# ghar1821/Chronoclust

Measured on AMD Instinct MI355X. Metric: points clustered/sec (20-dim), higher is better.
Workload: dtype f64; 1 GPU; C2: 1 timepoint, 1000000x20 synthetic blobs (seed 42+rank), 5000 microclusters; exact sequential semantics; online + offline phases per step; one independent st; points=1000000, dim=20, microclusters=5000, clusters=5000, streams=1

## Files before the change

chronoclust_amd/csrc/cc_api.hip:

```cpp
#include <hip/hip_runtime.h>

#include <algorithm>
#include <chrono>
#include <cmath>
#include <cstdio>
#include <cstdlib>
#include <cstring>
#include <limits>
#include <optional>
#include <string>
#include <thread>
#include <type_traits>
#include <vector>

#include "../../include/chronoclust_hip.h"
#include "cc_comm.h"
#include "cc_common.h"
#include "cc_csv.h"
#include "cc_offline.h"
#include "cc_online.h"
#include "cc_assign.h"
#include "cc_policy.h"
#include "cc_batch.h"

#include "cc_handle.h"

namespace {


template <int DP, bool DIRTY>
void launch_scan_dp(cc_handle* h, hipStream_t st, int win, Rows rows, const Cand* clean, Cand* part, int S, int round,
                    int mode, int shard_rank, int shard_world, int phase);

template <int DP>
int scan_u_wgs_per_cu()
{
    constexpr int NW = ScanShape<DP, false>::NW;
    static int blocks = 0;
    static const bool ok = hipOccupancyMaxActiveBlocksPerMultiprocessor(&blocks, k_scan_u<DP, NW>, 64 * NW, 0) == hipSuccess && blocks >= 1;
    return ok ? blocks : ScanUShape<DP>::WGS;
}

template <int DP>
ScanPlan scan_plan_dp(const cc_handle* h)
{
    ScanPlan p;
    p.dp = DP;
    const cc::ScanWidth w = cc::scan_width(h->d, h->hc.filter != 0, h->hc.pow2 != 0);
    p.scan_u = h->allow_scan_u && w.scan_u;
    p.pad_rows = p.scan_u && h->d != DP;
    if (p.scan_u && w.chain == CC_CHAIN_COMMON) p.chain = ScanPlan::COMMON;
    else if (h->allow_scan_p3 && h->allow_prune_general && !h->tainted && w.chain == CC_CHAIN_GENERAL) p.chain = ScanPlan::GENERAL;
    const bool p3 = h->allow_scan_p3 && DP <= 40;
    p.form = p3 ? ScanPlan::P3 : (h->allow_scan_p2 && DP <= 40 ? ScanPlan::P2 : ScanPlan::P1);
    if (p.chain == ScanPlan::COMMON && h->split_a_mode == 2) p.split_rows = 0;
    else if (p.chain == ScanPlan::COMMON && h->split_a_mode == 1 && !p3) p.split_rows = 10000;
    p.listed_rows = h->p3_listed_rows;
    const bool p3_sized = p3 && h->split_a_mode != 2;
    p.seed16 = h->allow_seed16 && (p.chain == ScanPlan::GENERAL || p3_sized);
    p.prune_applicable = p.chain != ScanPlan::NONE ? 1 : 0;
    p.allow_guess = (h->allow_guess && p.chain != ScanPlan::GENERAL) ? (h->allow_lean ? 1 : 2) : 0;
    p.allow_probe = (h->allow_probe && p.chain != ScanPlan::GENERAL) ? 1 : 0;
    p.force_prune_rows = (p.prune_applicable && h->allow_seed16 && p3_sized) ? h->force_prune_rows : 0;
    p.waves = ScanShape<DP, false>::NW;
    p.dirty_waves = ScanShape<DP, true>::NW;
    p.plain_wgs_per_cu = p.scan_u ? scan_u_wgs_per_cu<DP>() : ScanShape<DP, false>::WGS;
    p.prune_wgs_per_cu = h->prune_rounds4 > 0 ? h->prune_rounds4 : (DP <= 20 ? (p3_sized ? 8 : 16) : 24);
    return p;
}

ScanPlan scan_plan(const cc_handle* h)
{
    switch (cc::scan_width(h->d, false, false).padded) {
    case 4: return scan_plan_dp<4>(h);
    case 8: return scan_plan_dp<8>(h);
    case 14: return scan_plan_dp<14>(h);
    case 16: return scan_plan_dp<16>(h);
    case 20: return scan_plan_dp<20>(h);
    case 32: return scan_plan_dp<32>(h);
    case 40: return scan_plan_dp<40>(h);
    default: return scan_plan_dp<64>(h);
    }
}

template <int DP>
struct ScanCall {
    static constexpr int NW = ScanShape<DP, false>::NW;
    cc_handle* h; hipStream_t st; const Rows& rows;
    int round, mode, win, S;
    Cand* part;

    void scan_u(int n_pts, int srank, int sworld, const int* plist) const
    {
        hipLaunchKernelGGL((k_scan_u<DP, NW>), dim3((n_pts + 63) / 64, S), dim3(64 * NW), 0, st, h->ctl.p, h->Xt.p, rows.cen,
                           rows.scl, rows.kind, rows.key, part, round, mode, h->part_stride, srank, sworld, plist);
    }
    void prefix16() const
    {
        ensure_prefix16(h);
        const size_t a16_rows = h->tab.cap + 2 * CC_P16_TM;
        hipLaunchKernelGGL((k_prefix16<DP>), dim3((unsigned)((a16_rows + 255) / 256)), dim3(256), 0, st, (const Ctl*)h->ctl.p,
                           rows.cen, rows.kind, h->a16.p, h->hdr16.p, h->a16_stride, round, mode);
    }
    void seeds(int n_pts, int Sp, const int* plist, bool s16) const
    {
        const dim3 grid((n_pts + 127) / 128, Sp), block(64 * NW);
        if (s16) {
            if constexpr (DP <= 40) {
                hipLaunchKernelGGL((k_seed16<DP, NW>), grid, block, 0, st, (const Ctl*)h->ctl.p, (const double*)h->Xt.p, rows.cen, h->spart.p,
                                   round, mode, h->spart_stride, (const cc_h8*)h->a16.p, (const Prefix16Hdr*)h->hdr16.p, h->a16_stride);
                ++h->stats.seed16_launches;
            } else {
                throw HipErr{hipErrorInvalidValue, "k_seed16 is compiled up to 40 dimensions"};
            }
        } else {
            hipLaunchKernelGGL((k_seed<DP, NW>), grid, block, 0, st, h->ctl.p, h->Xt.p, rows.cen, rows.kind, h->spart.p, round, mode,
                               h->spart_stride, h->cmax.p, plist);
        }
        hipLaunchKernelGGL((k_seed_merge<DP>), dim3((2 * n_pts + 63) / 64), dim3(64), 0, st, h->ctl.p, h->X.p, rows.cen, rows.scl, h->spart.p,
                           h->spart_stride, Sp, h->thr.p, h->thr32.p, h->thr_stride, s16 ? 0.0 : h->prune_F, round, mode, h->cmax.p,
                           h->pstat_p(), plist, h->d);
    }
    template <bool LISTED, bool GENERAL>
    void scan_p3(unsigned lds, int srank, int sworld, double gF, unsigned long long* found) const
    {
        hipLaunchKernelGGL((k_scan_p3<DP, NW, LISTED, GENERAL>), dim3((win + 127) / 128, S), dim3(64 * NW), lds, st, h->ctl.p, h->Xt.p,
                           rows.cen, rows.scl, rows.kind, rows.key, h->thr.p, h->thr_stride, part, round, mode, h->part_stride, srank,
                           sworld, h->pstat_p(), gF, found, (const cc_h8*)h->a16.p, (const Prefix16Hdr*)h->hdr16.p, h->a16_stride,
                           GENERAL ? (const double*)h->X.p : nullptr, GENERAL ? rows.cf1 : nullptr, GENERAL ? rows.cf2 : nullptr,
                           GENERAL ? rows.w : nullptr);
    }
    void scan_p(int n_pts, int Sp, Cand* p, size_t p_stride, int srank, int sworld, const int* plist, double gF,
                unsigned long long* found) const
    {
        hipLaunchKernelGGL((k_scan_p<DP, NW, false>), dim3((n_pts + 63) / 64, Sp), dim3(64 * NW), 0, st, h->ctl.p, h->Xt.p, rows.cen,
                           rows.scl, rows.kind, rows.key, h->thr.p, h->thr32.p, h->thr_stride, p, round, mode, p_stride, srank, sworld,
                           h->pstat_p(), plist, gF, found, (const unsigned*)nullptr, (size_t)0, 0, 1);
    }
    void scan_split(int srank, int sworld, double gF, unsigned long long* found) const
    {
        const int nsub = S * NW;
        const int tps = cc_mask_tiles_per_sub((int)std::min<size_t>(h->tab.cap, (size_t)INT_MAX - 64), nsub);
        const size_t need = (size_t)((win + 127) / 128) * (size_t)nsub * (size_t)tps;
        if (need > h->mask_stride) { h->masks.ensure(2 * need); h->mask_stride = need; }
        hipLaunchKernelGGL((k_scan_a<DP, NW>), dim3((win + 127) / 128, S), dim3(64 * NW), 0, st, (const Ctl*)h->ctl.p,
                           (const double*)h->Xt.p, rows.cen, rows.kind, (const double*)h->thr.p, h->thr_stride, h->masks.p,
                           h->mask_stride, tps, round, mode, srank, sworld, gF);
        int q = 1;
        const int tiles = (win + 63) / 64;
        const int resident = h->n_cus * (DP <= 20 ? CC_SCANP_WGS20 : (DP <= 40 ? 3 : 2));
        for (int c = 1; c <= S; ++c)
            if (S % c == 0 && 2 * tiles * (S / c) >= 3 * resident) q = c;
        static const int q_env = []() { const char* e = getenv("CHRONOCLUST_HIP_SCANB_Q"); return e ? atoi(e) : 0; }();
        if (q_env > 0 && S % q_env == 0) q = q_env;
        hipLaunchKernelGGL((k_scan_p<DP, NW, true>), dim3(tiles, S / q), dim3(64 * NW), 0, st, h->ctl.p, h->Xt.p, rows.cen, rows.scl,
                           rows.kind, rows.key, h->thr.p, h->thr32.p, h->thr_stride, part, round, mode, h->part_stride, srank, sworld,
                           h->pstat_p(), (const int*)nullptr, gF, found, (const unsigned*)h->masks.p, h->mask_stride, tps, q);
    }
};

template <int DP, bool DIRTY>
void launch_scan_dp(cc_handle* h, hipStream_t st, int win, Rows rows, const Cand* clean, Cand* part, int S, int round,
                    int mode, int shard_rank, int shard_world, int phase)
{
    constexpr int NW = ScanShape<DP, DIRTY>::NW;
    const dim3 block(64 * NW);
    constexpr int TILE = 64 * ScanShape<DP, DIRTY>::PT;
    const dim3 grid((win + TILE - 1) / TILE, S);
    if constexpr (!DIRTY) {
        static_assert(ScanShape<DP, false>::PT == 1, "k_scan_u holds one window point per lane");
        const ScanPlan& pl = h->scan_plan;
        const ScanCall<DP> L{h, st, rows, round, mode, win, S, part};
        if (pl.scan_u) ++h->stats.scan_u_launches;
        if constexpr (DP > 8) {
            auto window_scan = [&](int srank, int sworld, double gF, unsigned long long* found, bool have_prefix16) {
                if (pl.split(h->hc.m_rows)) return L.scan_split(srank, sworld, gF, found);
                if constexpr (DP <= 40) {
                    if (pl.form == ScanPlan::P3) {
                        if (!have_prefix16) L.prefix16();
                        const bool listed = pl.listed(h->hc.m_rows);
                        if (pl.chain == ScanPlan::GENERAL) {
                            if (listed) L.template scan_p3<true, true>(0, srank, sworld, gF, found);
                            else L.template scan_p3<false, true>(0, srank, sworld, gF, found);
                        } else {
                            static const char* const lds_kb = getenv("CHRONOCLUST_HIP_SCAN_LDS_KB");
                            static const unsigned p3_lds = lds_kb ? (unsigned)atoi(lds_kb) * 1024u : 0u;
                            if (listed) L.template scan_p3<true, false>(p3_lds, srank, sworld, gF, found);
                            else L.template scan_p3<false, false>(p3_lds, srank, sworld, gF, found);
                        }
                        ++h->stats.scan_p2_launches;
                        return;
                    }
                    if (pl.form == ScanPlan::P2) {
                        hipLaunchKernelGGL((k_scan_p2<DP, NW>), dim3((win + 127) / 128, S), block, 0, st, h->ctl.p, h->Xt.p, rows.cen, rows.scl,
                                           rows.kind, rows.key, h->thr.p, h->thr_stride, part, round, mode, h->part_stride, srank, sworld,
                                           h->pstat_p(), gF, found);
                        ++h->stats.scan_p2_launches;
                        return;
                    }
                }
                L.scan_p(win, S, part, h->part_stride, srank, sworld, nullptr, gF, found);
            };
            auto seeded_chain = [&](int n_pts, const int* plist, Cand* p, size_t p_stride, int Sp, int srank, int sworld) {
                const bool whole_window = plist == nullptr && n_pts == win && p_stride == h->part_stride && Sp == S;
                const bool s16 = whole_window && pl.seed16;
                const bool have_prefix16 = whole_window && (s16 || pl.chain == ScanPlan::GENERAL);
                if constexpr (DP <= 40) if (have_prefix16) L.prefix16();
                L.seeds(n_pts, Sp, plist, s16);
                if (whole_window) window_scan(srank, sworld, 0.0, nullptr, have_prefix16);
                else L.scan_p(n_pts, Sp, p, p_stride, srank, sworld, plist, 0.0, nullptr);
            };
            auto missed_scan = [&](const int* list) {
                if (!h->allow_missed_plain) return seeded_chain(CC_MISSED_CAP, list, part, h->part_stride, S, shard_rank, shard_world);
                ++h->stats.missed_plain_launches;
                L.scan_u(CC_MISSED_CAP, shard_rank, shard_world, list);
            };
            if (pl.chain == ScanPlan::GENERAL && h->prune_now && phase == 0) {
                ++h->stats.scan_p_launches;
                return seeded_chain(win, nullptr, part, h->part_stride, S, shard_rank, shard_world);
            }
            if (pl.chain == ScanPlan::COMMON) {
                if (phase == 1) {
                    hipLaunchKernelGGL(k_missed_g, dim3(1), dim3(1024), 0, st, h->ctl.p, (const Cand*)h->gpart.p, h->gpart_stride,
                                       (size_t)win * 4 + 4, shard_world, h->missed.p, CC_MISSED_CAP, round, mode, h->found.p);
                    return missed_scan(h->missed.p);
                }
                if (!h->prune_now) {
                    L.scan_u(win, shard_rank, shard_world, nullptr);
                    if (!h->probe_now) return;
                    ++h->stats.probe_launches;
                    const int Sp = (int)std::max<size_t>(1, std::min<size_t>(128, h->spart_stride / 2 / 128));
                    h->probe_part.ensure((size_t)2 * 128 * Sp * 4);
                    return seeded_chain(std::min(win, 128), nullptr, h->probe_part.p, (size_t)128 * Sp * 4, Sp, 0, 1);
                }
                ++h->stats.scan_p_launches;
                if (!h->guess_now) return seeded_chain(win, nullptr, part, h->part_stride, S, shard_rank, shard_world);
                ++h->stats.scan_g_launches;
                unsigned long long* const found = h->lean_now ? nullptr : h->found.p;
                if (h->group_guess_now) {
                    hipLaunchKernelGGL(k_pstat_zero, dim3(1), dim3(2), 0, st, (const Ctl*)h->ctl.p, h->pstat_p(), round, mode);
                    return window_scan(shard_rank, shard_world, h->prune_F, found, false);
                }
                window_scan(0, 1, h->prune_F, found, false);
                if (h->lean_now) { ++h->stats.scan_lean_launches; return; }
                hipLaunchKernelGGL(k_missed, dim3(1), dim3(1024), 0, st, h->ctl.p, h->found.p, h->missed.p, CC_MISSED_CAP, round, mode);
                return missed_scan(h->missed.p);
            }
        }
        if (pl.scan_u) return L.scan_u(win, shard_rank, shard_world, nullptr);
    }
    const bool filter = DIRTY || h->hc.filter != 0;
#define CC_LAUNCH_SCAN(F, P) hipLaunchKernelGGL((k_scan<DP, F, P, DIRTY, NW>), grid, block, 0, st, h->ctl.p, h->X.p, h->Xt.p, rows, clean, \
                                          part, round, mode, h->part_stride, shard_rank, shard_world)
    if (filter) {
        if (h->hc.pow2) CC_LAUNCH_SCAN(true, true);
        else CC_LAUNCH_SCAN(true, false);
    } else if constexpr (!DIRTY) {
        if (h->hc.pow2) CC_LAUNCH_SCAN(false, true);
        else CC_LAUNCH_SCAN(false, false);
    }
#undef CC_LAUNCH_SCAN
}

template <bool DIRTY>
void launch_scan(cc_handle* h, hipStream_t st, int win, Rows rows, const Cand* clean, Cand* part, int S, int round,
                 int mode, int shard_rank = 0, int shard_world = 1, int phase = 0)
{
#define CC_SCAN_DP(DP) return launch_scan_dp<DP, DIRTY>(h, st, win, rows, clean, part, S, round, mode, shard_rank, shard_world, phase)
    switch (h->scan_plan.dp) {
    case 4: CC_SCAN_DP(4);
    case 8: CC_SCAN_DP(8);
    case 14: CC_SCAN_DP(14);
    case 16: CC_SCAN_DP(16);
    case 20: CC_SCAN_DP(20);
    case 32: CC_SCAN_DP(32);
    case 40: CC_SCAN_DP(40);
    case 64: CC_SCAN_DP(64);
    }
    throw HipErr{hipErrorInvalidValue, "launch_scan before scan_plan() (OnlineRun::prepare)"};
#undef CC_SCAN_DP
}

Rows padded_rows(cc_handle* h, hipStream_t st, Rows rows, int q, int round, int mode)
{
    const int dp = h->scan_plan.dp;
    ensure_pad_rows(h, dp);
    double* const cen = h->pad_cen.p + (size_t)q * h->pad_stride;
    double* const scl = h->pad_scl.p + (size_t)q * h->pad_stride;
    const dim3 grid((unsigned)((h->tab.cap * (size_t)(dp / 2) + 255) / 256));
#define CC_PAD_DP(DP) hipLaunchKernelGGL((k_pad_rows<DP>), grid, dim3(256), 0, st, (const Ctl*)h->ctl.p, rows.cen, rows.scl, cen, scl, \
                                         h->d, round, mode); break
    switch (dp) {
    case 14: CC_PAD_DP(14);
    case 16: CC_PAD_DP(16);
    case 20: CC_PAD_DP(20);
    case 32: CC_PAD_DP(32);
    case 40: CC_PAD_DP(40);
    case 64: CC_PAD_DP(64);
    default: throw HipErr{hipErrorInvalidValue, "padded_rows: no scan over padded operands at this width"};
    }
#undef CC_PAD_DP
    ++h->stats.pad_rows_launches;
    rows.cen = cen;
    rows.scl = scl;
    return rows;
}

}

#include "cc_online_run.h"
#include "cc_api_points.inc"
#include "cc_api_views.inc"
#include "cc_api_list.inc"
#include "cc_api_offline.inc"
#include "cc_api_comm.inc"
#include "cc_api_assign.inc"


extern "C" {

int cc_create(int device, cc_handle** out)
{
    if (!out) return CC_ERR_BAD_ARG;
    *out = nullptr;
    int ndev = 0;
    if (hipGetDeviceCount(&ndev) != hipSuccess || ndev <= 0 || device < 0 || device >= ndev) return CC_ERR_NO_DEVICE;
    cc_handle* h = new (std::nothrow) cc_handle();
    if (!h) return CC_ERR_OOM;
    h->device = device;
    int rc = guarded(h, [&]() {
        int prio_lo = 0, prio_hi = 0;
        int cus = 0;
        if (hipDeviceGetAttribute(&cus, hipDeviceAttributeMultiprocessorCount, device) == hipSuccess && cus > 0) h->n_cus = cus;
        HIPCHK(hipDeviceGetStreamPriorityRange(&prio_lo, &prio_hi));
        HIPCHK(hipStreamCreateWithPriority(&h->stream, hipStreamNonBlocking, prio_hi));
        HIPCHK(hipStreamCreateWithPriority(&h->stream2, hipStreamNonBlocking, prio_lo));
        h->ctl.ensure(1);
        if (hipHostMalloc((void**)&h->hc_pin, 2 * sizeof(Ctl), hipHostMallocDefault) != hipSuccess) h->hc_pin = nullptr;
        h->badflag.ensure(4);
        memset(&h->hc, 0, sizeof(Ctl));
        h->tun.window = CC_MAX_WINDOW;
        h->tun.rounds = 3;
        h->tun.segments = 64;
        h->tun.windows_per_sync = 16;
        h->tun.time_kernels = 0;
        read_knobs(*h);
        push_ctl(h);
        sync_stream(h, h->stream);
        return CC_OK;
    });
    if (rc != CC_OK) {
        delete h;
        return rc;
    }
    *out = h;
    return CC_OK;
}

void cc_destroy(cc_handle* h)
{
    if (!h) return;
    (void)hipSetDevice(h->device);
    if (h->pf.worker.joinable()) h->pf.worker.join();
    if (h->pf.stream) (void)hipStreamDestroy(h->pf.stream);
    if (h->hc_pin) (void)hipHostFree(h->hc_pin);
    for (int q = 0; q < 2; ++q)
        if (h->pf.pin[q]) (void)hipHostFree(h->pf.pin[q]);
    auto drain = [&](hipStream_t st) {
        if (!st) return;
        try {
            if (h->comm.rccl() && !h->comm.broken) h->comm.wait_stream(st);
            else (void)hipStreamSynchronize(st);
        } catch (const cc::CommErr&) {
        }
    };
    drain(h->stream);
    drain(h->stream2);
    h->comm.destroy();
    if (h->stream) {
        (void)hipStreamSynchronize(h->stream);
        (void)hipStreamDestroy(h->stream);
    }
    if (h->stream2) {
        (void)hipStreamSynchronize(h->stream2);
        (void)hipStreamDestroy(h->stream2);
    }
    for (hipEvent_t e : h->ev_pool) (void)hipEventDestroy(e);
    for (hipEvent_t e : h->sync_pool) (void)hipEventDestroy(e);
    delete h;
}

const char* cc_last_error(const cc_handle* h) { return h ? h->err.c_str() : "null handle"; }

int cc_set_tuning(cc_handle* h, const cc_tuning* t)
{
    if (!h || !t) return CC_ERR_BAD_ARG;
    if (t->window > 0) h->tun.window = std::min(t->window, CC_MAX_WINDOW);
    if (t->rounds > 0) h->tun.rounds = std::min(t->rounds, CC_MAX_ROUNDS);
    if (t->segments > 0) h->tun.segments = std::min(t->segments, 1024);
    if (t->windows_per_sync > 0) h->tun.windows_per_sync = t->windows_per_sync;
    h->tun.time_kernels = t->time_kernels;
    if (t->dirty_segments > 0) h->tun.dirty_segments = std::min(t->dirty_segments, 1024);
// ... 271 lines not shown
```

chronoclust_amd/csrc/cc_handle.h:

```cpp
#pragma once
#include "cc_knobs.h"

namespace {

struct HipErr {
    hipError_t e;
    const char* what;
};

#define HIPCHK(call)                                  \
    do {                                              \
        hipError_t _e = (call);                       \
        if (_e != hipSuccess) throw HipErr{_e, #call}; \
    } while (0)

template <typename T>
struct DevBuf {
    T* p = nullptr;
    size_t n = 0;
    void ensure(size_t count)
    {
        if (count <= n && p) return;
        release();
        size_t want = std::max<size_t>(count, 1);
        if (hipMalloc((void**)&p, want * sizeof(T)) != hipSuccess) {
            p = nullptr;
            throw HipErr{hipErrorOutOfMemory, "hipMalloc"};
        }
        n = want;
    }
    void release()
    {
        if (p) (void)hipFree(p);
        p = nullptr;
        n = 0;
    }
    ~DevBuf() { release(); }
    DevBuf() = default;
    DevBuf(const DevBuf&) = delete;
    DevBuf& operator=(const DevBuf&) = delete;
    DevBuf(DevBuf&& o) noexcept { swap(o); }
    DevBuf& operator=(DevBuf&& o) noexcept
    {
        if (this != &o) { release(); swap(o); }
        return *this;
    }
    void swap(DevBuf& o) noexcept
    {
        std::swap(p, o.p);
        std::swap(n, o.n);
    }
};

struct TableStore {
    DevBuf<double> cf1, cf2, cen, pref, scl, w;
    DevBuf<int> kind, key;
    DevBuf<long long> id, uid;
    DevBuf<unsigned long long> touch, last, carry_of, cnt;
    DevBuf<int> memb, clen, heavy;
    size_t cap = 0;
    int d = 0;
    enum Grow { KEPT, CLEARED, CLEARED_KEPT, SCRATCH };
    template <typename F>
    static void for_each_column(int dims, F&& f)
    {
        const size_t dim = (size_t)dims;
        f(&TableStore::cf1, dim, KEPT); f(&TableStore::cf2, dim, KEPT); f(&TableStore::cen, dim, KEPT);
        f(&TableStore::pref, dim, KEPT); f(&TableStore::scl, dim, KEPT);
        f(&TableStore::w, (size_t)1, KEPT); f(&TableStore::kind, (size_t)1, KEPT); f(&TableStore::key, (size_t)1, KEPT);
        f(&TableStore::id, (size_t)1, KEPT); f(&TableStore::uid, (size_t)1, KEPT);
        f(&TableStore::touch, (size_t)2, CLEARED); f(&TableStore::last, (size_t)2, CLEARED);
        f(&TableStore::carry_of, (size_t)1, CLEARED_KEPT);
        f(&TableStore::cnt, (size_t)1, CLEARED); f(&TableStore::memb, (size_t)CC_CHAIN_MEMB, SCRATCH);
        f(&TableStore::clen, (size_t)1, CLEARED);
        f(&TableStore::heavy, (size_t)1, CLEARED_KEPT);
    }
    void alloc(size_t rows, int dim)
    {
        for_each_column(dim, [&](auto col, size_t per_row, Grow) { (this->*col).ensure(rows * per_row); });
        cap = rows;
        d = dim;
    }
    Table view() const { return Table{cf1.p, cf2.p, cen.p, pref.p, scl.p, w.p, kind.p, key.p, id.p, uid.p, touch.p, last.p, carry_of.p, cnt.p, memb.p, clen.p, heavy.p, cap}; }
};

struct HostClusters {
    std::vector<int> mem, off{0};
    size_t size() const { return off.size() - 1; }
    void clear() { mem.clear(); off.assign(1, 0); }
};

}

struct PinArena {
    char* p = nullptr;
    size_t cap = 0, used = 0;
    void reset() { used = 0; }
    void reserve(size_t bytes)
    {
        if (bytes <= cap) return;
        if (p) (void)hipHostFree(p);
        p = nullptr;
        cap = 0;
        const size_t want = std::max<size_t>(bytes, (size_t)1 << 20);
        if (hipHostMalloc((void**)&p, want, hipHostMallocDefault) != hipSuccess) {
            p = nullptr;
            throw HipErr{hipErrorOutOfMemory, "hipHostMalloc"};
        }
        cap = want;
    }
    template <typename T>
    T* take(size_t n)
    {
        used = (used + 63) & ~(size_t)63;
        T* r = reinterpret_cast<T*>(p + used);
        used += std::max<size_t>(n, 1) * sizeof(T);
        if (used > cap) throw HipErr{hipErrorOutOfMemory, "page-locked scratch exhausted"};
        return r;
    }
    ~PinArena() { if (p) (void)hipHostFree(p); }
    PinArena() = default;
    PinArena(const PinArena&) = delete;
    PinArena& operator=(const PinArena&) = delete;
};

struct ScanPlan {
    int dp = 0;
    bool scan_u = false;
    bool pad_rows = false;
    enum Chain { NONE, COMMON, GENERAL } chain = NONE;
    enum Form { P3, P2, P1 } form = P1;
    long long split_rows = std::numeric_limits<long long>::max(), listed_rows = 0;
    bool seed16 = false;
    int prune_applicable = 0, allow_guess = 0, allow_probe = 0, force_prune_rows = 0;
    int waves = 4, dirty_waves = 4;
    int plain_wgs_per_cu = 1, prune_wgs_per_cu = 1;
    bool split(long long m_rows) const { return m_rows >= split_rows; }
    bool listed(long long m_rows) const { return m_rows >= listed_rows; }
};


struct BatchScanState {
    bool prune_now = false;
    bool group_guess_now = false;
    bool lean_now = false;
    bool guess_now = false;
    bool probe_now = false;
    ScanPlan scan_plan;
    void set_prune(int prune)
    {
        prune_now = prune != 0;
        guess_now = prune >= 2;
        lean_now = prune == 3;
    }
};

struct PrunedScanBuffers {
    DevBuf<Cand> probe_part;
    DevBuf<unsigned long long> found;
    DevBuf<int> missed;
    DevBuf<SeedCand> spart;
    DevBuf<double> thr;
    DevBuf<float> thr32;
    DevBuf<unsigned long long> cmax;
    DevBuf<cc_h8> a16;
    DevBuf<Prefix16Hdr> hdr16;
    size_t a16_stride = 0;
    DevBuf<unsigned> masks;
    size_t mask_stride = 0;
    DevBuf<double> pad_cen, pad_scl;
    size_t pad_stride = 0;
    size_t spart_stride = 0, thr_stride = 0;
};

struct WindowBuffers {
    int win_alloc = 0, seg_alloc = 0, d_alloc = 0;
    DevBuf<double> v_cf1, v_cf2, v_cen, v_pref, v_scl, v_w, v_dsq, v_tau;
    DevBuf<unsigned long long> v_tile_dsq;
    DevBuf<int> v_kind, v_key, v_next, v_upg, v_acc, v_tgt, v_skip, v_skip_car, v_unsafe;
    DevBuf<Cand> part, clean, dpart, dpart2, dseed;
    size_t part_stride = 0;
    DevBuf<double> c_cf1v, c_cf2v, c_cenv, c_prefv, c_sclv, c_wv, c_c0, c_w0, c_dsq;
    DevBuf<int> c_kind, c_key, c_slot, c_kind0;
    DevBuf<unsigned long long> c_tile_dsq;
    DevBuf<int> T0, T1, rk;
    DevBuf<int> link_near;
    DevBuf<int> sp_list;
    DevBuf<int> long_list;
    DevBuf<unsigned long long> lstat, lprev;
    bool prep_launched = false;
    DevBuf<CommitRec> rec;
    DevBuf<double> sh_cen[2], sh_scl[2], sh_cf1[2], sh_cf2[2], sh_w[2];
    DevBuf<int> sh_kind[2], sh_key[2];
    DevBuf<int8_t> dpath;
};

struct OfflineResults {
    DevBuf<double> pv_cf1, pv_cf2, pv_cen, pv_pref, pv_w, wvec;
    DevBuf<long long> pv_id;
    DevBuf<int> prow, nn, pdim, mem_dev, off_dev, nw_cnt, nw_nbr;
    DevBuf<long long> nw_off;
    DevBuf<int8_t> core;
    DevBuf<unsigned long long> adj, adjw;
    DevBuf<double> c_cf1, c_cf2, c_cen, c_pref, c_w;
    HostClusters clusters;
    PinArena pin;
    std::vector<long long> pcore_ids_host, pcore_uid_host;
    DevBuf<int32_t> pc_map, pc_out;
    int n_core = 0;
};

struct AssocScratch {
    DevBuf<double> a_cur_cen, a_cur_pref, a_prev_cen, a_dist, a_pdist;
    DevBuf<int> a_idx, a_pidx;
    DevBuf<int> flags;
};

struct RelaxedState {
    int relaxed_minibatch = 0;
    bool shard_suspended = false;
    DevBuf<double> rs_cf1, rs_cf2, rs_w, r_delta, r_gather;
    DevBuf<int> rs_kind, rs_key, r_didx, r_didx_all, r_cnt_all;
    DevBuf<long long> rs_id;
    DevBuf<double> rg_X, rg_Xt;
    DevBuf<long long> rg_uid;
    DevBuf<int8_t> rg_path;
    cc_relaxed_stats rstats{};
};

struct AssignBuffers {
    struct Set {
        DevBuf<double> X, Xt, dist;
        DevBuf<float> raw;
        DevBuf<long long> uid;
        DevBuf<int8_t> path;
        DevBuf<Cand> part;
        DevBuf<int> bad;
    } asg[2];
};

struct cc_handle : Knobs, BatchScanState, PrunedScanBuffers, WindowBuffers, OfflineResults, AssocScratch, RelaxedState, AssignBuffers {
    int device = 0;
    hipStream_t stream = nullptr;
    hipStream_t stream2 = nullptr;
    std::string err;
    cc_params par{};
    bool have_par = false;
    cc_tuning tun{};
    cc_stats stats{};

    int d = 0;
    TableStore tab, tab2;
    Ctl hc{};
    Ctl* hc_pin = nullptr;
    DevBuf<Ctl> ctl;
    unsigned long long* pstat_p() const { return (unsigned long long*)((char*)ctl.p + offsetof(Ctl, pstat)); }
    bool tainted = false;
    int adapt_win = 0;
    int clean_batches = 0;
    int since_shrink = 1000;
    DevBuf<int> seq_lists;
    DevBuf<double> seq_img;
    bool seq_sticky = false;
    int n_cus = 256;

    DevBuf<double> X, Xt;
    long long n_points = 0;
    double x_absmax = 0.0;
    DevBuf<long long> lab_uid;
    DevBuf<int8_t> lab_path;
    DevBuf<int> badflag;
    DevBuf<double> scr, scr2;
    DevBuf<float> ingest_raw[2];
    long long f32_points = 0;
    long long view_points = 0;
    long long list_points = 0;
    DevBuf<int> list_desc;

    struct Prefetch {
        std::thread worker;
        bool active = false;
        const void* x = nullptr;
        long long n = 0;
        int d = 0;
        bool scaled = false;
        bool f32 = false;
        long long piece = 0;
        bool view = false;
        int dtype = 0;
        long long rs = 0, cs = 0;
        bool list = false;
        int src_cols = 0, flags = 0;
        std::vector<cc_list_desc> ldesc;
        DevBuf<int> desc;
        DevBuf<float> raw[2];
        std::vector<double> scale, mn;
        DevBuf<double> X, Xt, sm;
        DevBuf<int> bad;
        hipStream_t stream = nullptr;
        void* pin[2] = {nullptr, nullptr};
        size_t pin_bytes = 0;
        int bad_host[4] = {0, 0, 0, 0};
        int rc = 0;
        const char* what = "";
    } pf;

    std::vector<hipEvent_t> ev_pool, sync_pool;

    cc::Comm comm;
    long long shard_min_row_dims = 400000;
    long long shard_min_row_dims_pruned = 0;
    double calib_ag_us = 0.0, calib_scan_ns = 0.0;
    int offline_shard_min_rows = 8192;
// ... 271 lines not shown
```

chronoclust_amd/csrc/cc_scan.h:

```cpp
#pragma once


#define CC_SCAN_TM 16
#ifndef CC_SCAN_PT_CLEAN
#define CC_SCAN_PT_CLEAN 1
#endif
#ifndef CC_SCAN_WGS_CLEAN
#define CC_SCAN_WGS_CLEAN 4
#endif
#ifndef CC_SCAN_WGS_CLEAN40
#define CC_SCAN_WGS_CLEAN40 3
#endif
#ifndef CC_SCAN_WGS_DIRTY32
#define CC_SCAN_WGS_DIRTY32 3
#endif
#ifndef CC_SCAN_NW_CLEAN
#define CC_SCAN_NW_CLEAN 4
#endif
template <int DP, bool DIRTY>
struct ScanShape {
    static constexpr int PT = (!DIRTY && DP == 20) ? CC_SCAN_PT_CLEAN : 1;
    static constexpr int NW = (!DIRTY && DP == 20) ? CC_SCAN_NW_CLEAN : 4;
    static constexpr int WGS = (!DIRTY && DP == 20) ? CC_SCAN_WGS_CLEAN
                               : (DP <= 20 ? 4 : (DP <= 40 ? (DIRTY ? CC_SCAN_WGS_DIRTY32 : (DP == 40 ? CC_SCAN_WGS_CLEAN40 : 3)) : 2));
// ... 365 lines not shown
            const bool liveB = RB2 ? row_bounds(m + 1, kindB, boundB) : false;
            if (!liveA && !liveB) continue;

            double accA[PT], accB[PT];
#pragma unroll
            for (int t = 0; t < PT; ++t) { accA[t] = 0.0; accB[t] = 0.0; }
            bool alive = true;
            const int mB = (m + 1 < CC_SCAN_TM) ? m + 1 : m;
#pragma unroll
            for (int i0 = 0; i0 < DP; i0 += 4) {
#pragma unroll
                for (int q = 0; q < 4; ++q) {
                    const int i = i0 + q;
                    if (i < DP) {
                        const double cA = s_c_base[m * DP + i], sA = s_s_base[m * DP + i];
                        const double cB = s_c_base[mB * DP + i], sB = s_s_base[mB * DP + i];
#pragma unroll
                        for (int t = 0; t < PT; ++t) {
                            double x = p[t][i] - cA;
                            x = x * x;
                            if (FUSE) accA[t] = __builtin_fma(x, sA, accA[t]);
                            else {
                                x = POW2 ? x * sA : x / sA;
                                accA[t] = accA[t] + x;
                            }
                            if (RB2) {
                                double y = p[t][i] - cB;
                                y = y * y;
                                if (FUSE) accB[t] = __builtin_fma(y, sB, accB[t]);
                                else {
                                    y = POW2 ? y * sB : y / sB;
                                    accB[t] = accB[t] + y;
                                }
                            }
                        }
                    }
                }
                if (i0 + 4 < DP) {
                    bool q = false;
#pragma unroll
                    for (int t = 0; t < PT; ++t) q = q || (accA[t] <= boundA[t]) || (RB2 && accB[t] <= boundB[t]);
                    if (__builtin_amdgcn_ballot_w64(q) == 0ull) {
                        alive = false;
                        break;
                    }
                }
            }
            if (!alive) continue;

            auto insert_row = [&](int mm, int kind, const double (&acc)[PT], const double (&bound)[PT]) {
                const int rowg = rt + mm;
                const int rowc = carried ? CC_CAR_BASE + rowg : rowg;
                const int key = s_key_w[mm];
#pragma unroll
                for (int t = 0; t < PT; ++t) {
                    if (!(acc[t] <= bound[t])) continue;
                    auto consider = [&](auto KC) {
                        constexpr int K = decltype(KC)::value;
                        constexpr int R = DIRTY ? 0 : 1;
                        if (!cand_less(acc[t], key, bd[K][t][R], bk[K][t][R])) return;
                        if (K == 0 && filter) {
                            int ne1 = 0;
                            cc_tentative_radius(rows.cf1 + (size_t)rowg * d, rows.cf2 + (size_t)rowg * d,
                                                rows.w[rowg], X + (cursor + jj[t]) * d, d, par, nullptr, &ne1);
                            if (ne1 > par.pi) return;
                        }
                        if (cand_less(acc[t], key, bd[K][t][0], bk[K][t][0])) {
                            bd[K][t][1] = bd[K][t][0]; bk[K][t][1] = bk[K][t][0]; bs[K][t][1] = bs[K][t][0];
                            bd[K][t][0] = acc[t]; bk[K][t][0] = key; bs[K][t][0] = rowc;
                        } else {
                            bd[K][t][1] = acc[t]; bk[K][t][1] = key; bs[K][t][1] = rowc;
                        }
                    };
                    if (kind == 0) consider(std::integral_constant<int, 0>{});
                    else consider(std::integral_constant<int, 1>{});
                }
            };
            if (liveA) insert_row(m, kindA, accA, boundA);
            if (RB2 && liveB) insert_row(m + 1, kindB, accB, boundB);
        }
        };
        if (POW2 && fuse_tile) dirty_rows(std::true_type{});
        else dirty_rows(std::false_type{});
    }

    if (!DIRTY) {
#pragma unroll
        for (int kd = 0; kd < 2; ++kd)
#pragma unroll
            for (int t = 0; t < PT; ++t)
#pragma unroll
                for (int r = 0; r < 2; ++r) bk[kd][t][r] = bs[kd][t][r] >= 0 ? rows.key[bs[kd][t][r]] : CC_IDX_INF;
    }
    Cand* const s_m = reinterpret_cast<Cand*>(smem);
    auto s_m_at = [&](int w, int t, int c) -> Cand& { return s_m[((w * PT + t) * 4 + c) * 64 + lane]; };
    __syncthreads();
    if (wv > 0) {
#pragma unroll
        for (int t = 0; t < PT; ++t) {
            s_m_at(wv - 1, t, 0) = Cand{bd[0][t][0], bk[0][t][0], bs[0][t][0]};
            s_m_at(wv - 1, t, 1) = Cand{bd[0][t][1], bk[0][t][1], bs[0][t][1]};
            s_m_at(wv - 1, t, 2) = Cand{bd[1][t][0], bk[1][t][0], bs[1][t][0]};
            s_m_at(wv - 1, t, 3) = Cand{bd[1][t][1], bk[1][t][1], bs[1][t][1]};
        }
    }
    __syncthreads();
    if (wv != 0) return;
#pragma unroll
    for (int t = 0; t < PT; ++t) {
        if (!valid[t]) continue;
        Cand c0{bd[0][t][0], bk[0][t][0], bs[0][t][0]}, c1{bd[0][t][1], bk[0][t][1], bs[0][t][1]};
        Cand c2{bd[1][t][0], bk[1][t][0], bs[1][t][0]}, c3{bd[1][t][1], bk[1][t][1], bs[1][t][1]};
#pragma unroll
        for (int w = 0; w < NW - 1; ++w) {
            cc_top2_push(c0, c1, s_m_at(w, t, 0));
            cc_top2_push(c0, c1, s_m_at(w, t, 1));
            cc_top2_push(c2, c3, s_m_at(w, t, 2));
            cc_top2_push(c2, c3, s_m_at(w, t, 3));
        }
        if (DIRTY) {
            Cand* o = part + ((size_t)jj[t] * S + blockIdx.y) * 2;
            o[0] = c0;
            o[1] = c2;
        } else {
            Cand* o = part + ((size_t)jj[t] * S + blockIdx.y) * 4;
            o[0] = c0; o[1] = c1; o[2] = c2; o[3] = c3;
        }
    }
    }
}

#ifndef CC_SCANU_WGS40
#define CC_SCANU_WGS40 4
#endif
template <int DP>
struct ScanUShape {
    static constexpr int WGS = DP <= 32 ? 4 : (DP <= 40 ? CC_SCANU_WGS40 : 2);
};
template <int BIT>
__device__ __forceinline__ void cc_sel_scale2(unsigned mask, double scaled, double one, double& o0, double& o1)
{
    asm("s_bitcmp1_b32 %2, %3\n\ts_cselect_b64 %0, %5, %6\n\ts_bitcmp1_b32 %2, %4\n\ts_cselect_b64 %1, %5, %6"
        : "=&s"(o0), "=&s"(o1)
        : "s"(mask), "n"(BIT), "n"(BIT + 1), "s"(scaled), "s"(one)
        : "scc");
}

__device__ __forceinline__ int cc_after(int row, double dep)
{
    asm("" : "+s"(row) : "v"(dep));
    return row;
}

template <int DP, int NW>
__global__ __launch_bounds__(64 * NW, ScanUShape<DP>::WGS) void k_scan_u(const Ctl* __restrict__ ctl, const double* __restrict__ Xt,
                                                                 const double* __restrict__ g_cen,
                                                                 const double* __restrict__ g_scl,
                                                                 const int* __restrict__ g_kind,
                                                                 const int* __restrict__ g_key, Cand* __restrict__ part,
                                                                 int round, int mode, size_t part_stride, int shard_rank,
                                                                 int shard_world, const int* __restrict__ plist = nullptr)
{
    static_assert(DP % 2 == 0 && DP >= 4 && DP <= 64, "padded dimensionalities are even");
    constexpr int NP = DP / 2;
    constexpr int NC = 2 * ((NP + 9) / 10);
    constexpr int CH_MAX = 2 * ((NP + NC - 1) / NC);
    int B, m_rows_scan, q;
    long long cursor;
    if (mode == 1) {
        q = round & 1;
        B = ctl->la_b[q];
        m_rows_scan = ctl->la_rows[q];
        cursor = ctl->la_cursor[q];
    } else {
        B = ctl->win_b;
        m_rows_scan = ctl->m_rows;
        cursor = ctl->cursor;
        if (ctl->mode != 0) return;
        q = (int)(ctl->window_seq & 1ull);
    }
    part += (size_t)q * part_stride;
    if (B == 0) return;
    if (plist) plist += (size_t)q * CC_MISSED_CAP;
    const int n_here = plist ? ctl->n_missed[q] : B;
    const int j0 = (int)blockIdx.x * 64;
    if (j0 >= n_here) return;
    const int lane = threadIdx.x & 63;
    const int wv = __builtin_amdgcn_readfirstlane(threadIdx.x >> 6);
    const int S = gridDim.y;
    const int nsub = S * NW;
    const int sub = blockIdx.y * NW + wv;
    int row_lo = 0, row_hi = m_rows_scan;
    if (shard_world > 1) cc_shard_range(m_rows_scan, shard_world, shard_rank, 1, &row_lo, &row_hi);
    const int nrows = row_hi - row_lo;
    const int per = (nrows + nsub - 1) / nsub;
    const int r0 = row_lo + sub * per;
    const int r1 = min(row_hi, r0 + per);
    const size_t n_pts = (size_t)ctl->xt_stride;
    const double k = ctl->k;
    const double inv_k = ctl->inv_k;
    const bool valid = j0 + lane < n_here;
    const int jj = plist ? (valid ? plist[j0 + lane] : 0) : j0 + lane;

    double p[DP];
    {
        const double* xp = Xt + cursor + (valid ? jj : 0);
#pragma unroll
        for (int i = 0; i < DP; ++i) p[i] = valid ? xp[(size_t)i * n_pts] : 0.0;
    }
    bool fuse_wave = k >= 0x1p-64 && k <= 0x1p64;
    {
        bool tn = false;
#pragma unroll
        for (int i = 0; i < DP; ++i) tn = tn || cc_is_tiny(p[i]);
        fuse_wave = fuse_wave && __builtin_amdgcn_ballot_w64(tn) == 0ull;
    }
    double bd[2][2];
    int bs[2][2];
#pragma unroll
    for (int kd = 0; kd < 2; ++kd)
#pragma unroll
        for (int r = 0; r < 2; ++r) {
            bd[kd][r] = valid ? CC_INF : -CC_INF;
            bs[kd][r] = -1;
        }

    for (int rt = r0; rt < r1; rt += CC_SCAN_TM) {
        const int tm = __builtin_amdgcn_readfirstlane(min(CC_SCAN_TM, r1 - rt));
        double buf[2][CH_MAX];
        {
            const double* __restrict__ c0 = g_cen + (size_t)rt * DP;
#pragma unroll
            for (int i = 0; i < 2 * (NP / NC); ++i) buf[0][i] = c0[i];
        }
        constexpr int NL = (CC_SCAN_TM * DP + 63) / 64;
        int rm_lo = 0, rm_hi = 0;
        bool fuse_tile;
        {
            const double* gc = g_cen + (size_t)rt * DP;
            const double* gs = g_scl + (size_t)rt * DP;
            unsigned long long rmask = 0ull;
            bool tn = false;
            const int off = (lane & (CC_SCAN_TM - 1)) * DP;
#pragma unroll
            for (int q = 0; q < NL; ++q) {
                const int e = lane + q * 64;
                const bool in = e < tm * DP;
                const double tc = in ? gc[e] : 0.0;
                const double ts = in ? gs[e] : 1.0;
                tn = tn || cc_is_tiny(tc);
                const unsigned long long w = __builtin_amdgcn_ballot_w64(ts != 1.0);
                const int rel = off - 64 * q;
                const unsigned long long a = (rel >= 0 && rel < 64) ? (w >> (rel & 63)) : 0ull;
                const unsigned long long b = (rel < 0 && rel > -DP) ? (w << ((-rel) & 63)) : 0ull;
                rmask |= a | b;
            }
            if (DP < 64) rmask &= (1ull << (DP & 63)) - 1ull;
            rm_lo = (int)(unsigned)(rmask & 0xFFFFFFFFull);
            rm_hi = (int)(unsigned)(rmask >> 32);
            fuse_tile = fuse_wave && __builtin_amdgcn_ballot_w64(tn) == 0ull;
        }
        unsigned pmask, omask;
        {
            const int kd = (lane < tm) ? g_kind[rt + lane] : CC_KIND_DEAD;
            pmask = (unsigned)__builtin_amdgcn_ballot_w64(kd == CC_KIND_PCORE);
            omask = (unsigned)__builtin_amdgcn_ballot_w64(kd == CC_KIND_OUTLIER);
        }
        auto rows_of_tile = [&](auto FUSEC, auto KSELC) {
            constexpr bool FUSE = decltype(FUSEC)::value;
            constexpr int KSEL = decltype(KSELC)::value;
            for (int m = 0; m < tm; ++m) {
                const unsigned mlo = (unsigned)__builtin_amdgcn_readlane(rm_lo, m);
                const unsigned mhi = (DP > 32) ? (unsigned)__builtin_amdgcn_readlane(rm_hi, m) : 0u;
                const int rowg = rt + m;
                const int rown = min(rowg + 1, rt + tm - 1);
                const double one = 1.0;
                double acc = 0.0;
                auto pair_step = [&](auto IC, double c0, double c1, double x0) {
                    constexpr int i = decltype(IC)::value;
                    double s0, s1;
                    cc_sel_scale2<(i & 31)>(i < 32 ? mlo : mhi, inv_k, one, s0, s1);
                    double x = x0;
                    double y = p[i + 1] - c1;
                    x = x * x;
                    y = y * y;
                    if (FUSE) {
                        acc = (i == 0) ? x * s0 : __builtin_fma(x, s0, acc);
                        acc = __builtin_fma(y, s1, acc);
                    } else {
                        x = x * s0;
                        y = y * s1;
                        acc = (i == 0) ? x : acc + x;
                        acc = acc + y;
                    }
                };
                cc_static_for<NC>([&](auto CC) {
                    constexpr int c = decltype(CC)::value;
                    constexpr int lo = 2 * (c * NP / NC), hi = 2 * ((c + 1) * NP / NC);
                    constexpr int cn = (c + 1) % NC;
                    constexpr int nlo = 2 * (cn * NP / NC), nhi = 2 * ((cn + 1) * NP / NC);
                    const double x0 = p[lo] - buf[c & 1][0];
                    const double* __restrict__ nx = g_cen + (size_t)cc_after(c + 1 < NC ? rowg : rown, x0) * DP;
#pragma unroll
                    for (int i = 0; i < nhi - nlo; ++i) buf[cn & 1][i] = nx[nlo + i];
                    cc_static_for<(hi - lo) / 2>([&](auto QC) {
                        constexpr int i = 2 * decltype(QC)::value;
                        pair_step(std::integral_constant<int, lo + i>{}, buf[c & 1][i], buf[c & 1][i + 1],
                                  (i == 0) ? x0 : p[lo + i] - buf[c & 1][i]);
                    });
                });
                auto update = [&](auto KC) {
                    constexpr int K = decltype(KC)::value;
                    const double a = acc;
                    double& d0 = bd[K][0];
                    double& d1 = bd[K][1];
                    int& s0 = bs[K][0];
                    int& s1 = bs[K][1];
                    bool ins = a < d1;
                    bool first = a < d0;
                    const unsigned long long e1 = __builtin_amdgcn_ballot_w64(a == d1);
                    const unsigned long long e0 = __builtin_amdgcn_ballot_w64(a == d0);
                    if ((e1 | e0) != 0ull) {
                        if (a == d1 || a == d0) {
                            const int key = g_key[rowg];
                            if (a == d1) ins = key < (s1 >= 0 ? g_key[s1] : CC_IDX_INF);
                            if (a == d0) first = key < (s0 >= 0 ? g_key[s0] : CC_IDX_INF);
                        }
                    }
                    d1 = cc_vmin(d1, cc_vmax(d0, a));
                    d0 = cc_vmin(d0, a);
                    s1 = first ? s0 : (ins ? rowg : s1);
                    s0 = first ? rowg : s0;
                };
                if constexpr (KSEL == 0) update(std::integral_constant<int, 0>{});
                else if constexpr (KSEL == 1) update(std::integral_constant<int, 1>{});
                else {
                    if ((pmask >> m) & 1u) update(std::integral_constant<int, 0>{});
                    else if ((omask >> m) & 1u) update(std::integral_constant<int, 1>{});
                }
            }
        };
        const unsigned full = (1u << tm) - 1u;
        if (fuse_tile) {
            if (pmask == full) rows_of_tile(std::true_type{}, std::integral_constant<int, 0>{});
            else if (omask == full) rows_of_tile(std::true_type{}, std::integral_constant<int, 1>{});
            else rows_of_tile(std::true_type{}, std::integral_constant<int, -1>{});
        } else rows_of_tile(std::false_type{}, std::integral_constant<int, -1>{});
    }

    int bk[2][2];
#pragma unroll
    for (int kd = 0; kd < 2; ++kd)
#pragma unroll
        for (int r = 0; r < 2; ++r) bk[kd][r] = bs[kd][r] >= 0 ? g_key[bs[kd][r]] : CC_IDX_INF;
    __shared__ Cand s_m[(NW > 1 ? NW - 1 : 1) * 4 * 64];
    auto s_m_at = [&](int w, int c) -> Cand& { return s_m[(w * 4 + c) * 64 + lane]; };
    if (wv > 0) {
        s_m_at(wv - 1, 0) = Cand{bd[0][0], bk[0][0], bs[0][0]};
        s_m_at(wv - 1, 1) = Cand{bd[0][1], bk[0][1], bs[0][1]};
        s_m_at(wv - 1, 2) = Cand{bd[1][0], bk[1][0], bs[1][0]};
        s_m_at(wv - 1, 3) = Cand{bd[1][1], bk[1][1], bs[1][1]};
    }
    __syncthreads();
    if (wv != 0 || !valid) return;
    Cand c0{bd[0][0], bk[0][0], bs[0][0]}, c1{bd[0][1], bk[0][1], bs[0][1]};
    Cand c2{bd[1][0], bk[1][0], bs[1][0]}, c3{bd[1][1], bk[1][1], bs[1][1]};
#pragma unroll
    for (int w = 0; w < NW - 1; ++w) {
        cc_top2_push(c0, c1, s_m_at(w, 0));
        cc_top2_push(c0, c1, s_m_at(w, 1));
        cc_top2_push(c2, c3, s_m_at(w, 2));
        cc_top2_push(c2, c3, s_m_at(w, 3));
    }
    Cand* o = part + ((size_t)jj * S + blockIdx.y) * 4;
    o[0] = c0; o[1] = c1; o[2] = c2; o[3] = c3;
}


struct __attribute__((aligned(8))) SeedCand {
    float part;
    int row;
};

struct ScanWin {
    int B, rows, q;
    long long cursor;
};
__device__ __forceinline__ ScanWin cc_scan_window(const Ctl* __restrict__ ctl, int round, int mode)
{
    ScanWin w;
    if (mode == 1) {
        w.q = round & 1;
        w.B = ctl->la_b[w.q];
        w.rows = ctl->la_rows[w.q];
        w.cursor = ctl->la_cursor[w.q];
    } else {
        w.B = (ctl->mode != 0) ? 0 : ctl->win_b;
        w.rows = ctl->m_rows;
        w.cursor = ctl->cursor;
        w.q = (int)(ctl->window_seq & 1ull);
    }
    return w;
}

template <int DP>
__global__ __launch_bounds__(256) void k_pad_rows(const Ctl* __restrict__ ctl, const double* __restrict__ g_cen,
                                                  const double* __restrict__ g_scl, double* __restrict__ m_cen,
                                                  double* __restrict__ m_scl, int d, int round, int mode)
{
    static_assert(DP % 2 == 0, "padded dimensionalities are even");
    constexpr int HP = DP / 2;
    const ScanWin win = cc_scan_window(ctl, round, mode);
    if (win.B == 0) return;
    const size_t t = (size_t)blockIdx.x * 256 + threadIdx.x;
    const size_t row = t / HP;
    if (row >= (size_t)win.rows) return;
    const int i = 2 * (int)(t % HP);
    const double* __restrict__ c = g_cen + row * (size_t)d;
    const double* __restrict__ s = g_scl + row * (size_t)d;
    double2 vc, vs;
    vc.x = (i < d) ? c[i] : 0.0;
    vc.y = (i + 1 < d) ? c[i + 1] : 0.0;
    vs.x = (i < d) ? s[i] : 1.0;
    vs.y = (i + 1 < d) ? s[i + 1] : 1.0;
    *reinterpret_cast<double2*>(m_cen + 2 * t) = vc;
    *reinterpret_cast<double2*>(m_scl + 2 * t) = vs;
}

typedef float cc_f2 __attribute__((ext_vector_type(2)));
typedef float cc_f4 __attribute__((ext_vector_type(4)));
#define CC_PRE 8

template <int DP>
__device__ __forceinline__ void cc_load_prefix(const double* __restrict__ g_cen, const int* __restrict__ g_kind, int rt,
                                               int tm, int lane, double (&tc)[2], int& kd)
{
#pragma unroll
    for (int q = 0; q < 2; ++q) {
        const int e = lane + q * 64, m = e >> 3, i = e & 7;
        tc[q] = (m < tm) ? g_cen[(size_t)(rt + m) * DP + i] : 0.0;
    }
    kd = (lane < tm) ? g_kind[rt + lane] : CC_KIND_DEAD;
}

__device__ __forceinline__ float cc_prefix_score(const cc_f2 (&p2)[CC_PRE / 2], const cc_f4* __restrict__ row)
{
    const cc_f4 c01 = row[0], c23 = row[1];
    cc_f2 x0 = p2[0] - cc_f2{c01.x, c01.y};
    cc_f2 x1 = p2[1] - cc_f2{c01.z, c01.w};
    cc_f2 x2 = p2[2] - cc_f2{c23.x, c23.y};
    cc_f2 x3 = p2[3] - cc_f2{c23.z, c23.w};
    cc_f2 acc = x0 * x0;
    acc = __builtin_elementwise_fma(x1, x1, acc);
    acc = __builtin_elementwise_fma(x2, x2, acc);
    acc = __builtin_elementwise_fma(x3, x3, acc);
    return acc.x + acc.y;
}

template <int DP, int NW>
__global__ __launch_bounds__(64 * NW, 4) void k_seed(const Ctl* __restrict__ ctl, const double* __restrict__ Xt,
                                                   const double* __restrict__ g_cen, const int* __restrict__ g_kind,
                                                   SeedCand* __restrict__ spart, int round, int mode, size_t spart_stride,
                                                   unsigned long long* __restrict__ cmax, const int* __restrict__ plist)
{
    static_assert(CC_PRE == 8 && CC_PRE <= DP, "prefix dimensions");
    const ScanWin win = cc_scan_window(ctl, round, mode);
    const int B = win.B;
    if (B == 0) return;
    const int j0 = (int)blockIdx.x * 128;
    if (plist) plist += (size_t)win.q * CC_MISSED_CAP;
    const int n_pts_here = plist ? ctl->n_missed[win.q] : B;
    if (j0 >= n_pts_here) return;
    spart += (size_t)win.q * spart_stride;
    const int lane = threadIdx.x & 63;
    const int wv = __builtin_amdgcn_readfirstlane(threadIdx.x >> 6);
    const int S = gridDim.y;
    const int nsub = S * NW;
    const int sub = blockIdx.y * NW + wv;
    const int per = (win.rows + nsub - 1) / nsub;
    const int r0 = sub * per;
    const int r1 = min(win.rows, r0 + per);
    const size_t n_pts = (size_t)ctl->xt_stride;
    double org[CC_PRE];
#pragma unroll
    for (int i = 0; i < CC_PRE; ++i) org[i] = g_cen[i];
    int jj[2];
    bool valid[2];
    cc_f2 p2[2][CC_PRE / 2];
#pragma unroll
    for (int u = 0; u < 2; ++u) {
        const int e = j0 + u * 64 + lane;
        valid[u] = e < n_pts_here;
        jj[u] = plist ? (valid[u] ? plist[e] : 0) : e;
        const double* xp = Xt + win.cursor + (valid[u] ? jj[u] : 0);
#pragma unroll
        for (int i = 0; i < CC_PRE / 2; ++i)
            p2[u][i] = cc_f2{valid[u] ? (float)(xp[(size_t)(2 * i) * n_pts] - org[2 * i]) : 0.f,
                             valid[u] ? (float)(xp[(size_t)(2 * i + 1) * n_pts] - org[2 * i + 1]) : 0.f};
    }
    __shared__ __attribute__((aligned(16))) float s_pre[NW * CC_SCAN_TM * CC_PRE];
    __shared__ float s_h[NW * CC_SCAN_TM];
    float* const tile = s_pre + (size_t)wv * CC_SCAN_TM * CC_PRE;
    float* const th = s_h + (size_t)wv * CC_SCAN_TM;
    float best[2][2];
    int idx[2][2];
#pragma unroll
    for (int u = 0; u < 2; ++u)
#pragma unroll
        for (int K = 0; K < 2; ++K) { best[u][K] = -__builtin_inff(); idx[u][K] = -1; }
    double tc[2];
    int kdl = CC_KIND_DEAD;
    double cm = 0.0;
    if (r0 < r1) cc_load_prefix<DP>(g_cen, g_kind, r0, min(CC_SCAN_TM, r1 - r0), lane, tc, kdl);
    for (int rt = r0; rt < r1; rt += CC_SCAN_TM) {
        const int tm = __builtin_amdgcn_readfirstlane(min(CC_SCAN_TM, r1 - rt));
        CC_WAVE_SYNC();
#pragma unroll
        for (int q = 0; q < 2; ++q) {
            cm = __builtin_fmax(cm, __builtin_fabs(tc[q]));
            const float v = (float)(tc[q] - org[lane & 7]);
            tile[lane + q * 64] = v;
            float hsum = v * v;
            hsum += __shfl_xor(hsum, 1);
            hsum += __shfl_xor(hsum, 2);
            hsum += __shfl_xor(hsum, 4);
            if ((lane & 7) == 0) th[(lane >> 3) + q * 8] = 0.5f * hsum;
        }
        const unsigned pmask = (unsigned)__builtin_amdgcn_ballot_w64(kdl == CC_KIND_PCORE);
// ... 1167 lines not shown
```

Before: 77.77 million points/s.

## Scan missed-point list with row-split grid and shuffle merge kernel

Replaces the plain scan over the missed-point list with a dedicated kernel, k_scan_ul. It puts row shards on grid x, up to 64 slices sized from the row count, and missed-point tiles on grid y, then writes partial top-2 candidates to a separate list buffer. A new merge kernel reduces the slices per missed point with wave shuffles and scatters the result into the main partition array, filling the unused slots with sentinels. The aim is more parallelism over microcluster rows for the small missed set, at the cost of an extra launch, a new buffer and a merge pass.

```diff
diff --git a/chronoclust_amd/csrc/cc_api.hip b/chronoclust_amd/csrc/cc_api.hip
--- a/chronoclust_amd/csrc/cc_api.hip
+++ b/chronoclust_amd/csrc/cc_api.hip
@@ -90,10 +90,21 @@
     int round, mode, win, S;
     Cand* part;
 
-    void scan_u(int n_pts, int srank, int sworld, const int* plist) const
+    void scan_u(int srank, int sworld) const
     {
-        hipLaunchKernelGGL((k_scan_u<DP, NW>), dim3((n_pts + 63) / 64, S), dim3(64 * NW), 0, st, h->ctl.p, h->Xt.p, rows.cen,
-                           rows.scl, rows.kind, rows.key, part, round, mode, h->part_stride, srank, sworld, plist);
+        hipLaunchKernelGGL((k_scan_u<DP, NW>), dim3((win + 63) / 64, S), dim3(64 * NW), 0, st, h->ctl.p, h->Xt.p, rows.cen,
+                           rows.scl, rows.kind, rows.key, part, round, mode, h->part_stride, srank, sworld);
+    }
+    void scan_list(int srank, int sworld, const int* plist) const
+    {
+        const size_t rows_here = (size_t)h->hc.m_rows / (size_t)std::max(1, sworld) + 1;
+        const int SL = (int)std::min<size_t>(CC_LIST_SL_MAX, (rows_here + CC_SCAN_TM * NW - 1) / (CC_SCAN_TM * NW));
+        const size_t lstride = (size_t)CC_MISSED_CAP * CC_LIST_SL_MAX * 4;
+        h->list_part.ensure(2 * lstride);
+        hipLaunchKernelGGL((k_scan_ul<DP, NW>), dim3(SL, CC_MISSED_CAP / 64), dim3(64 * NW), 0, st, h->ctl.p, h->Xt.p, rows.cen,
+                           rows.scl, rows.kind, rows.key, h->list_part.p, round, mode, lstride, srank, sworld, plist);
+        hipLaunchKernelGGL(k_merge_list, dim3(CC_MISSED_CAP / 4), dim3(256), 0, st, (const Ctl*)h->ctl.p, (const Cand*)h->list_part.p,
+                           lstride, SL, part, h->part_stride, S, round, mode, plist);
     }
     void prefix16() const
     {
@@ -213,7 +224,7 @@
             auto missed_scan = [&](const int* list) {
                 if (!h->allow_missed_plain) return seeded_chain(CC_MISSED_CAP, list, part, h->part_stride, S, shard_rank, shard_world);
                 ++h->stats.missed_plain_launches;
-                L.scan_u(CC_MISSED_CAP, shard_rank, shard_world, list);
+                L.scan_list(shard_rank, shard_world, list);
             };
             if (pl.chain == ScanPlan::GENERAL && h->prune_now && phase == 0) {
                 ++h->stats.scan_p_launches;
@@ -226,7 +237,7 @@
                     return missed_scan(h->missed.p);
                 }
                 if (!h->prune_now) {
-                    L.scan_u(win, shard_rank, shard_world, nullptr);
+                    L.scan_u(shard_rank, shard_world);
                     if (!h->probe_now) return;
                     ++h->stats.probe_launches;
                     const int Sp = (int)std::max<size_t>(1, std::min<size_t>(128, h->spart_stride / 2 / 128));
@@ -247,7 +258,7 @@
                 return missed_scan(h->missed.p);
             }
         }
-        if (pl.scan_u) return L.scan_u(win, shard_rank, shard_world, nullptr);
+        if (pl.scan_u) return L.scan_u(shard_rank, shard_world);
     }
     const bool filter = DIRTY || h->hc.filter != 0;
 #define CC_LAUNCH_SCAN(F, P) hipLaunchKernelGGL((k_scan<DP, F, P, DIRTY, NW>), grid, block, 0, st, h->ctl.p, h->X.p, h->Xt.p, rows, clean, \
diff --git a/chronoclust_amd/csrc/cc_handle.h b/chronoclust_amd/csrc/cc_handle.h
--- a/chronoclust_amd/csrc/cc_handle.h
+++ b/chronoclust_amd/csrc/cc_handle.h
@@ -159,6 +159,7 @@
     DevBuf<Cand> probe_part;
     DevBuf<unsigned long long> found;
     DevBuf<int> missed;
+    DevBuf<Cand> list_part;
     DevBuf<SeedCand> spart;
     DevBuf<double> thr;
     DevBuf<float> thr32;
diff --git a/chronoclust_amd/csrc/cc_scan.h b/chronoclust_amd/csrc/cc_scan.h
--- a/chronoclust_amd/csrc/cc_scan.h
+++ b/chronoclust_amd/csrc/cc_scan.h
@@ -541,14 +541,13 @@
     return row;
 }
 
-template <int DP, int NW>
-__global__ __launch_bounds__(64 * NW, ScanUShape<DP>::WGS) void k_scan_u(const Ctl* __restrict__ ctl, const double* __restrict__ Xt,
-                                                                 const double* __restrict__ g_cen,
-                                                                 const double* __restrict__ g_scl,
-                                                                 const int* __restrict__ g_kind,
-                                                                 const int* __restrict__ g_key, Cand* __restrict__ part,
-                                                                 int round, int mode, size_t part_stride, int shard_rank,
-                                                                 int shard_world, const int* __restrict__ plist = nullptr)
+template <int DP, int NW, bool LIST>
+__device__ __forceinline__ void cc_scan_u_body(const Ctl* __restrict__ ctl, const double* __restrict__ Xt,
+                                               const double* __restrict__ g_cen, const double* __restrict__ g_scl,
+                                               const int* __restrict__ g_kind, const int* __restrict__ g_key,
+                                               Cand* __restrict__ part, int round, int mode, size_t part_stride, int shard_rank,
+                                               int shard_world, const int* __restrict__ plist, const int tile, const int y,
+                                               const int n_y)
 {
     static_assert(DP % 2 == 0 && DP >= 4 && DP <= 64, "padded dimensionalities are even");
     constexpr int NP = DP / 2;
@@ -570,15 +569,15 @@
     }
     part += (size_t)q * part_stride;
     if (B == 0) return;
-    if (plist) plist += (size_t)q * CC_MISSED_CAP;
-    const int n_here = plist ? ctl->n_missed[q] : B;
-    const int j0 = (int)blockIdx.x * 64;
+    if (LIST) plist += (size_t)q * CC_MISSED_CAP;
+    const int n_here = LIST ? ctl->n_missed[q] : B;
+    const int j0 = tile * 64;
     if (j0 >= n_here) return;
     const int lane = threadIdx.x & 63;
     const int wv = __builtin_amdgcn_readfirstlane(threadIdx.x >> 6);
-    const int S = gridDim.y;
+    const int S = n_y;
     const int nsub = S * NW;
-    const int sub = blockIdx.y * NW + wv;
+    const int sub = y * NW + wv;
     int row_lo = 0, row_hi = m_rows_scan;
     if (shard_world > 1) cc_shard_range(m_rows_scan, shard_world, shard_rank, 1, &row_lo, &row_hi);
     const int nrows = row_hi - row_lo;
@@ -589,7 +588,7 @@
     const double k = ctl->k;
     const double inv_k = ctl->inv_k;
     const bool valid = j0 + lane < n_here;
-    const int jj = plist ? (valid ? plist[j0 + lane] : 0) : j0 + lane;
+    const int jj = LIST ? (valid ? plist[j0 + lane] : 0) : j0 + lane;
 
     double p[DP];
     {
@@ -761,8 +760,78 @@
         cc_top2_push(c2, c3, s_m_at(w, 2));
         cc_top2_push(c2, c3, s_m_at(w, 3));
     }
-    Cand* o = part + ((size_t)jj * S + blockIdx.y) * 4;
+    Cand* o = part + ((size_t)(LIST ? j0 + lane : jj) * S + y) * 4;
     o[0] = c0; o[1] = c1; o[2] = c2; o[3] = c3;
+}
+
+template <int DP, int NW>
+__global__ __launch_bounds__(64 * NW, ScanUShape<DP>::WGS) void k_scan_u(const Ctl* __restrict__ ctl, const double* __restrict__ Xt,
+                                                                 const double* __restrict__ g_cen,
+                                                                 const double* __restrict__ g_scl,
+                                                                 const int* __restrict__ g_kind,
+                                                                 const int* __restrict__ g_key, Cand* __restrict__ part,
+                                                                 int round, int mode, size_t part_stride, int shard_rank,
+                                                                 int shard_world)
+{
+    cc_scan_u_body<DP, NW, false>(ctl, Xt, g_cen, g_scl, g_kind, g_key, part, round, mode, part_stride, shard_rank, shard_world,
+                                  nullptr, (int)blockIdx.x, (int)blockIdx.y, (int)gridDim.y);
+}
+
+#define CC_LIST_SL_MAX 64
+
+template <int DP, int NW>
+__global__ __launch_bounds__(64 * NW, ScanUShape<DP>::WGS) void k_scan_ul(const Ctl* __restrict__ ctl, const double* __restrict__ Xt,
+                                                                  const double* __restrict__ g_cen,
+                                                                  const double* __restrict__ g_scl,
+                                                                  const int* __restrict__ g_kind,
+                                                                  const int* __restrict__ g_key, Cand* __restrict__ lpart,
+                                                                  int round, int mode, size_t lpart_stride, int shard_rank,
+                                                                  int shard_world, const int* __restrict__ plist)
+{
+    cc_scan_u_body<DP, NW, true>(ctl, Xt, g_cen, g_scl, g_kind, g_key, lpart, round, mode, lpart_stride, shard_rank, shard_world,
+                                 plist, (int)blockIdx.y, (int)blockIdx.x, (int)gridDim.x);
+}
+
+__global__ __launch_bounds__(256) void k_merge_list(const Ctl* __restrict__ ctl, const Cand* __restrict__ lpart, size_t lpart_stride,
+                                                    int SL, Cand* __restrict__ part, size_t part_stride, int S, int round, int mode,
+                                                    const int* __restrict__ plist)
+{
+    int B, q;
+    if (mode == 1) {
+        q = round & 1;
+        B = ctl->la_b[q];
+    } else {
+        B = ctl->win_b;
+        if (ctl->mode != 0) return;
+        q = (int)(ctl->window_seq & 1ull);
+    }
+    const int e = (int)blockIdx.x * 4 + (int)(threadIdx.x >> 6);
+    if (B == 0 || e >= ctl->n_missed[q]) return;
+    const int lane = threadIdx.x & 63;
+    const Cand none = Cand{CC_INF, CC_IDX_INF, -1};
+    Cand c0 = none, c1 = none, c2 = none, c3 = none;
+    if (lane < SL) {
+        const Cand* src = lpart + (size_t)q * lpart_stride + ((size_t)e * SL + lane) * 4;
+        c0 = src[0]; c1 = src[1]; c2 = src[2]; c3 = src[3];
+    }
+    auto other = [](const Cand& c, int w) { return Cand{__shfl_xor(c.dist, w, 64), __shfl_xor(c.key, w, 64), __shfl_xor(c.slot, w, 64)}; };
+#pragma unroll
+    for (int w = 1; w < 64; w <<= 1) {
+        const Cand x0 = other(c0, w), x1 = other(c1, w), x2 = other(c2, w), x3 = other(c3, w);
+        cc_top2_push(c0, c1, x0);
+        cc_top2_push(c0, c1, x1);
+        cc_top2_push(c2, c3, x2);
+        cc_top2_push(c2, c3, x3);
+    }
+    const int j = plist[(size_t)q * CC_MISSED_CAP + e];
+    Cand* o = part + (size_t)q * part_stride + (size_t)j * S * 4;
+    for (int s = lane; s < S; s += 64) {
+        const bool first = s == 0;
+        o[(size_t)s * 4 + 0] = first ? c0 : none;
+        o[(size_t)s * 4 + 1] = first ? c1 : none;
+        o[(size_t)s * 4 + 2] = first ? c2 : none;
+        o[(size_t)s * 4 + 3] = first ? c3 : none;
+    }
 }
 
 
```

Measured after the change: 78.71 million points/s (median of 6 runs). +1.2%, better.
